# wesselb/stheno

Hardware: NVIDIA H100
Metric: log-marginal-likelihoods/sec (n=16384 fp64 EQ) (higher is better)
Workload: dtype f64

## Files before the change

stheno_b200/csrc/common.cuh:

```cuda
#pragma once
#include <cuda_runtime.h>
#include <stdint.h>

#include <atomic>
#include <mutex>

#include "../../include/gpk.h"

namespace gpk {

extern long long g_launch_count;

#define GPK_CHECK_LAUNCH()                                   \
  do {                                                       \
    cudaError_t e__ = cudaGetLastError();                    \
    if (e__ != cudaSuccess) return -1000 - (int)e__;         \
  } while (0)

#define GPK_COUNT_LAUNCH() (++::gpk::g_launch_count)

template <auto Kernel>
int opt_in_smem(int bytes) {
  static std::atomic<int> set[64];
  static std::mutex mu;
  int dev = 0;
  cudaError_t e = cudaGetDevice(&dev);
  if (e != cudaSuccess) return -1000 - (int)e;
  if (dev >= 64) return GPK_ERR_UNSUPPORTED;
  if (bytes <= set[dev].load(std::memory_order_acquire)) return 0;
  std::lock_guard<std::mutex> lock(mu);
  if (bytes <= set[dev].load(std::memory_order_relaxed)) return 0;
  e = cudaFuncSetAttribute(Kernel, cudaFuncAttributeMaxDynamicSharedMemorySize, bytes);
  if (e != cudaSuccess) return -1000 - (int)e;
  set[dev].store(bytes, std::memory_order_release);
  return 0;
}

__device__ __forceinline__ uint32_t smem_u32(const void* p) {
  return static_cast<uint32_t>(__cvta_generic_to_shared(p));
}

__device__ __forceinline__ void cp_async16(void* smem_dst, const void* gmem_src) {
  asm volatile("cp.async.cg.shared.global [%0], [%1], 16;\n" ::"r"(smem_u32(smem_dst)), "l"(gmem_src));
}
__device__ __forceinline__ void cp_async_commit() { asm volatile("cp.async.commit_group;\n" ::); }
template <int N>
__device__ __forceinline__ void cp_async_wait() {
  asm volatile("cp.async.wait_group %0;\n" ::"n"(N));
}

__device__ __forceinline__ void mbar_init(uint64_t* bar, uint32_t count) {
  asm volatile("mbarrier.init.shared::cta.b64 [%0], %1;\n" ::"r"(smem_u32(bar)), "r"(count));
}
__device__ __forceinline__ void fence_mbar_init() { asm volatile("fence.mbarrier_init.release.cluster;\n" ::); }
__device__ __forceinline__ void fence_proxy_async() { asm volatile("fence.proxy.async.shared::cta;\n" ::); }
__device__ __forceinline__ void mbar_arrive_expect_tx(uint64_t* bar, uint32_t bytes) {
  asm volatile("mbarrier.arrive.expect_tx.shared::cta.b64 _, [%0], %1;\n" ::"r"(smem_u32(bar)), "r"(bytes));
}
__device__ __forceinline__ void mbar_wait(uint64_t* bar, uint32_t phase) {
  asm volatile(
      "{\n"
      ".reg .pred P1;\n"
      "WAIT_LOOP:\n"
      "mbarrier.try_wait.parity.shared::cta.b64 P1, [%0], %1;\n"
      "@P1 bra WAIT_DONE;\n"
      "bra WAIT_LOOP;\n"
      "WAIT_DONE:\n"
      "}\n" ::"r"(smem_u32(bar)),
      "r"(phase)
      : "memory");
}
__device__ __forceinline__ void bulk_copy_g2s(void* smem_dst, const void* gmem_src, uint32_t bytes, uint64_t* bar) {
  asm volatile(
      "cp.async.bulk.shared::cluster.global.mbarrier::complete_tx::bytes [%0], [%1], %2, [%3];\n" ::"r"(
          smem_u32(smem_dst)),
      "l"(gmem_src), "r"(bytes), "r"(smem_u32(bar))
      : "memory");
}

__device__ __forceinline__ void dmma884(double& c0, double& c1, double a, double b) {
  asm("mma.sync.aligned.m8n8k4.row.col.f64.f64.f64.f64 {%0,%1}, {%2}, {%3}, {%0,%1};\n"
               : "+d"(c0), "+d"(c1)
               : "d"(a), "d"(b));
}

struct Emulation {
  int32_t slices = 0;
  void* scratch = nullptr;
  int64_t bytes = 0;
};
Emulation& emulation();

template <typename T>
__device__ __forceinline__ T warp_sum(T v) {
#pragma unroll
  for (int o = 16; o > 0; o >>= 1) v += __shfl_xor_sync(0xffffffffu, v, o);
  return v;
}

}
```

stheno_b200/csrc/gemm_oz.cu:

```cuda
#include <cuda.h>

#include "common.cuh"
#include "wgmma.cuh"

namespace gpk {
bool prof_enabled();
void prof_begin(cudaStream_t, double flops, int kind);
void prof_end(cudaStream_t);

namespace {

constexpr int OZ_BM = 128, OZ_BN = 64, OZ_BK = 64;
constexpr int OZ_HN = 32;
constexpr int OZ_THREADS = 384;

template <int S>
struct OzCfg {
  static constexpr bool PAD = S > 7;
  static constexpr int EXTRA = PAD ? 0 : S / 2;
  static constexpr int ACC = 16 * (S + EXTRA);
  static constexpr int RA = (192 - ACC) / 8 < S ? (192 - ACC) / 8 : S;
  static constexpr int A_SLICE = OZ_BM * OZ_BK;
  static constexpr int B_SLICE = OZ_HN * OZ_BK;
  static constexpr int A_BYTES = S * A_SLICE;
  static constexpr int Z_BYTES = PAD ? B_SLICE : 0;
  static constexpr int B_BYTES = S * B_SLICE;
  static constexpr int TX_BYTES = A_BYTES + B_BYTES;
  static constexpr int STAGE_BYTES = A_BYTES + Z_BYTES + B_BYTES;
  static constexpr int SMEM_MAX = 226 * 1024;
  static constexpr int STAGES = (SMEM_MAX - 1024) / STAGE_BYTES > 4 ? 4 : (SMEM_MAX - 1024) / STAGE_BYTES;
  static constexpr int SMEM_BYTES = STAGES * STAGE_BYTES + 1024;
  static_assert(STAGES >= 2, "ring");
};

struct OzParams {
  double alpha;
  double* C;
  const double* sc_a;
  const double* sc_b;
  int64_t ldc;
  int32_t a_row0, b_row0;
  int32_t KB, lower, tiles_m, tiles_n;
  int32_t total_tiles, tiles_per_cta, tri_rows;
  int32_t accumulate;
  int32_t band;
};

__device__ __forceinline__ void oz_mbar_wait(uint64_t* bar, uint32_t parity) {
  asm volatile(
      "{\n"
      ".reg .pred P1;\n"
      "OZW_LOOP:\n"
      "mbarrier.try_wait.parity.shared::cta.b64 P1, [%0], %1;\n"
      "@P1 bra OZW_DONE;\n"
      "bra OZW_LOOP;\n"
      "OZW_DONE:\n"
      "}\n" ::"r"(smem_u32(bar)),
      "r"(parity)
      : "memory");
}
__device__ __forceinline__ void oz_mbar_arrive(uint64_t* bar) {
  asm volatile("mbarrier.arrive.shared::cta.b64 _, [%0];\n" ::"r"(smem_u32(bar)) : "memory");
}
__device__ __forceinline__ void oz_tma_load_3d(void* dst, const CUtensorMap* map, int c0, int c1, int c2, uint64_t* bar) {
  asm volatile(
      "cp.async.bulk.tensor.3d.shared::cluster.global.mbarrier::complete_tx::bytes [%0], [%1, {%2, %3, %4}], [%5];\n" ::"r"(
          smem_u32(dst)),
      "l"(map), "r"(c0), "r"(c1), "r"(c2), "r"(smem_u32(bar))
      : "memory");
}
__device__ __forceinline__ double oz_i2d(uint32_t x) {
  return __hiloint2double(0x43300000, (int)(x ^ 0x80000000u)) - 4503601774854144.0;
}
template <int S, int SA, int N>
__device__ __forceinline__ void oz_wgmma(uint32_t* d, const uint32_t* a, uint32_t a_addr, uint32_t b_addr, uint32_t accumulate) {
  if constexpr (SA < OzCfg<S>::RA)
    wgmma_s8_ra<N>(d, a + 4 * SA, wgmma_desc<64>(b_addr), accumulate);
  else
    wgmma_s8<N>(d, wgmma_desc<64>(a_addr + SA * OzCfg<S>::A_SLICE), wgmma_desc<64>(b_addr), accumulate);
}
template <int S, int SA, int LO>
__device__ __forceinline__ void oz_mma_groups(uint32_t* acc, const uint32_t* a, uint32_t a_addr, uint32_t b_addr,
                                              uint32_t accumulate) {
  constexpr int W = S - LO < 2 ? S - LO : 2;
  oz_wgmma<S, SA, OZ_HN * W>(acc + 16 * LO, a, a_addr, b_addr + (LO - SA) * OzCfg<S>::B_SLICE, accumulate);
  if constexpr (LO + 2 < S) oz_mma_groups<S, SA, LO + 2>(acc, a, a_addr, b_addr, accumulate);
}
template <int S, int SA>
__device__ __forceinline__ void oz_mma_step(uint32_t* acc, const uint32_t* a, uint32_t a_addr, uint32_t b_addr,
                                            uint32_t accumulate) {
  using Cfg = OzCfg<S>;
  if constexpr (SA & 1) {
    if constexpr (Cfg::PAD)
      oz_wgmma<S, SA, 2 * OZ_HN>(acc + 16 * (SA - 1), a, a_addr, b_addr - Cfg::B_SLICE, 1u);
    else
      oz_wgmma<S, SA, OZ_HN>(acc + 16 * (S + SA / 2), a, a_addr, b_addr, accumulate);
  }
  constexpr int LO = (SA + 1) & ~1;
  if constexpr (LO < S) oz_mma_groups<S, SA, LO>(acc, a, a_addr, b_addr, SA == 0 ? accumulate : 1u);
  if constexpr (SA + 1 < S) oz_mma_step<S, SA + 1>(acc, a, a_addr, b_addr, accumulate);
}
__host__ __device__ __forceinline__ int oz_rows_before(const OzParams& p, int r) {
  if (!p.lower) return r * p.tiles_n;
  return r <= p.tri_rows ? r * (r + 1) : p.tri_rows * (p.tri_rows + 1) + (r - p.tri_rows) * p.tiles_n;
}
__host__ __device__ __forceinline__ void oz_tile(const OzParams& p, int t, int& tm, int& tn) {
  int r0 = 0;
  while (r0 + p.band < p.tiles_m && oz_rows_before(p, r0 + p.band) <= t) r0 += p.band;
  const int r1 = (r0 + p.band < p.tiles_m) ? r0 + p.band : p.tiles_m;
  int u = t - oz_rows_before(p, r0);
  const int nc0 = (p.lower && 2 * (r0 + 1) < p.tiles_n) ? 2 * (r0 + 1) : p.tiles_n;
  const int h = r1 - r0;
  if (u < nc0 * h) {
    tn = u / h;
    tm = r0 + (u - tn * h);
    return;
  }
  u -= nc0 * h;
  for (int c = nc0; c < p.tiles_n; ++c) {
    const int first = (c >> 1) > r0 ? (c >> 1) : r0;
    const int cnt = r1 - first;
    if (u < cnt) {
      tn = c;
      tm = first + u;
      return;
    }
    u -= cnt;
  }
  tm = r1 - 1;
  tn = p.tiles_n - 1;
}

template <int S>
__global__ void __launch_bounds__(OZ_THREADS, 1)
oz_gemm_kernel(const __grid_constant__ CUtensorMap mapA, const __grid_constant__ CUtensorMap mapB, const OzParams p) {
  using Cfg = OzCfg<S>;
  constexpr int STAGES = Cfg::STAGES;
  const int wg = threadIdx.x >> 7;
  const int t_begin = blockIdx.x * p.tiles_per_cta;
  const int t_end = min(t_begin + p.tiles_per_cta, p.total_tiles);

  extern __shared__ uint8_t oz_smem_raw[];
  uint8_t* smem = reinterpret_cast<uint8_t*>((reinterpret_cast<uintptr_t>(oz_smem_raw) + 1023) & ~uintptr_t(1023));
  __shared__ __align__(8) uint64_t full_bar[STAGES], empty_bar[STAGES];

  if (threadIdx.x == 0) {
    for (int s = 0; s < STAGES; ++s) {
      mbar_init(&full_bar[s], 1);
      mbar_init(&empty_bar[s], 256);
    }
    fence_mbar_init();
  }
  if constexpr (Cfg::PAD) {
    for (int i = threadIdx.x; i < STAGES * Cfg::Z_BYTES / 16; i += OZ_THREADS) {
      const int st = i / (Cfg::Z_BYTES / 16), j = i % (Cfg::Z_BYTES / 16);
      reinterpret_cast<uint4*>(smem + st * Cfg::STAGE_BYTES + Cfg::A_BYTES)[j] = make_uint4(0, 0, 0, 0);
    }
    asm volatile("fence.proxy.async.shared::cta;\n" ::: "memory");
  }
  __syncthreads();
  const int KB = p.KB;

  if (wg == 0) {
    asm volatile("setmaxnreg.dec.sync.aligned.u32 40;\n" ::);
    if (threadIdx.x == 0) {
      int g = 0;
      for (int t = t_begin; t < t_end; ++t) {
        int tm, tn;
        oz_tile(p, t, tm, tn);
        for (int h = 0; h < 2; ++h) {
          for (int kb = 0; kb < KB; ++kb, ++g) {
            const int s = g % STAGES, it = g / STAGES;
            if (it > 0) oz_mbar_wait(&empty_bar[s], (it - 1) & 1);
            uint8_t* st = smem + s * Cfg::STAGE_BYTES;
            mbar_arrive_expect_tx(&full_bar[s], Cfg::TX_BYTES);
            oz_tma_load_3d(st, &mapA, kb * OZ_BK, p.a_row0 + tm * OZ_BM, 0, &full_bar[s]);
            oz_tma_load_3d(st + Cfg::A_BYTES + Cfg::Z_BYTES, &mapB, kb * OZ_BK, p.b_row0 + tn * OZ_BN + h * OZ_HN, 0, &full_bar[s]);
          }
        }
      }
    }
    return;
  }
  asm volatile("setmaxnreg.inc.sync.aligned.u32 232;\n" ::);
  const int tid = threadIdx.x - 128 * wg, wrow = 64 * (wg - 1);
  const int r_lo = 16 * (tid >> 5) + ((tid & 31) >> 2), c_lo = 2 * (tid & 3);
  const double w_last = __hiloint2double((1023 - (12 + 7 * (S - 1))) << 20, 0);
  const int lane = tid & 31, a_row = wrow + 16 * (tid >> 5) + (lane & 7) + 8 * ((lane >> 3) & 1);
  const uint32_t a_off0 = a_row * OZ_BK + ((((lane >> 4) + 0) ^ ((lane >> 1) & 3)) << 4);
  const uint32_t a_off1 = a_row * OZ_BK + ((((lane >> 4) + 2) ^ ((lane >> 1) & 3)) << 4);
  uint32_t acc[Cfg::ACC];
  int g = 0;
  for (int t = t_begin; t < t_end; ++t) {
    int tm, tn;
    oz_tile(p, t, tm, tn);
    for (int h = 0; h < 2; ++h) {
      for (int kb = 0; kb < KB; ++kb, ++g) {
        const int s = g % STAGES, it = g / STAGES;
        oz_mbar_wait(&full_bar[s], it & 1);
        const uint32_t st = smem_u32(smem + s * Cfg::STAGE_BYTES), b0 = st + Cfg::A_BYTES + Cfg::Z_BYTES;
        uint32_t a[2][4 * Cfg::RA];
#pragma unroll
        for (int sl = 0; sl < Cfg::RA; ++sl) {
          ldmatrix_x4(a[0] + 4 * sl, st + sl * Cfg::A_SLICE + a_off0);
          ldmatrix_x4(a[1] + 4 * sl, st + sl * Cfg::A_SLICE + a_off1);
        }
        wgmma_fence();
#pragma unroll
        for (int ks = 0; ks < 2; ++ks)
          oz_mma_step<S, 0>(acc, a[ks], st + wrow * OZ_BK + ks * 32, b0 + ks * 32, (kb > 0 || ks > 0) ? 1u : 0u);
        wgmma_commit();
        wgmma_wait<0>();
        oz_mbar_arrive(&empty_bar[s]);
      }
      if constexpr (Cfg::EXTRA > 0) {
#pragma unroll
        for (int d = 1; d < S; d += 2)
#pragma unroll
          for (int i = 0; i < 16; ++i) acc[16 * d + i] += acc[16 * (S + d / 2) + i];
      }
      const int64_t row0 = (int64_t)tm * OZ_BM + wrow + r_lo;
      const int64_t col0 = (int64_t)tn * OZ_BN + h * OZ_HN + c_lo;
#pragma unroll
      for (int i = 0; i < 16; ++i) {
        const int64_t row = row0 + 8 * ((i >> 1) & 1), col = col0 + 8 * (i >> 2) + (i & 1);
        double v = oz_i2d(acc[i]);
#pragma unroll
        for (int d = 1; d < S; ++d) v = fma(v, 128.0, oz_i2d(acc[16 * d + i]));
        const double rs = p.alpha * w_last * __ldg(p.sc_a + row);
        const double out = v * (rs * __ldg(p.sc_b + col));
        double* c = p.C + row * p.ldc + col;
        if (p.accumulate)
          atomicAdd(c, out);
        else
          *c = out;
      }
    }
  }
}

template <int S>
__global__ void __launch_bounds__(256)
oz_slice_kernel(const double* __restrict__ P, int64_t ldp, int64_t rows, int32_t K, int8_t* __restrict__ planes,
                int64_t plane_stride, double* __restrict__ sc) {
  const int64_t row = (int64_t)blockIdx.x * 8 + (threadIdx.x >> 5);
  const int lane = threadIdx.x & 31;
  if (row >= rows) return;
  const double* src = P + row * ldp;
  double m = 0.0;
  for (int k = lane * 4; k < K; k += 128) {
    const double2 a = *reinterpret_cast<const double2*>(src + k), b = *reinterpret_cast<const double2*>(src + k + 2);
    m = fmax(fmax(fabs(a.x), fabs(a.y)), fmax(m, fmax(fabs(b.x), fabs(b.y))));
  }
#pragma unroll
  for (int o = 16; o > 0; o >>= 1) m = fmax(m, __shfl_xor_sync(0xffffffffu, m, o));
  int e = 0;
  if (m > 0.0 && m < 1e300) {
    e = ilogb(m) + 1;
    e = max(-1000, min(1000, e));
  }
  const double inv = __hiloint2double((1023 - e) << 20, 0);
  if (lane == 0) sc[row] = __hiloint2double((1023 + e) << 20, 0);
  int8_t* dst = planes + row * K;
  for (int k = lane * 4; k < K; k += 128) {
    const double2 a = *reinterpret_cast<const double2*>(src + k), b = *reinterpret_cast<const double2*>(src + k + 2);
    double r[4] = {a.x * inv, a.y * inv, b.x * inv, b.y * inv};
    double pw = 64.0, ipw = 1.0 / 64.0;
#pragma unroll
    for (int s = 0; s < S; ++s) {
      char4 q;
      double t;
      t = rint(r[0] * pw); r[0] = fma(-t, ipw, r[0]); q.x = (signed char)(int)t;
      t = rint(r[1] * pw); r[1] = fma(-t, ipw, r[1]); q.y = (signed char)(int)t;
      t = rint(r[2] * pw); r[2] = fma(-t, ipw, r[2]); q.z = (signed char)(int)t;
      t = rint(r[3] * pw); r[3] = fma(-t, ipw, r[3]); q.w = (signed char)(int)t;
      *reinterpret_cast<char4*>(dst + (int64_t)s * plane_stride + k) = q;
      pw *= 128.0;
      ipw *= 1.0 / 128.0;
    }
  }
}

typedef CUresult (*OzEncodeTiledFn)(CUtensorMap*, CUtensorMapDataType, cuuint32_t, void*, const cuuint64_t*,
                                    const cuuint64_t*, const cuuint32_t*, const cuuint32_t*, CUtensorMapInterleave,
                                    CUtensorMapSwizzle, CUtensorMapL2promotion, CUtensorMapFloatOOBfill);
OzEncodeTiledFn oz_encode_fn() {
  static OzEncodeTiledFn fn = [] {
    void* p = nullptr;
    cudaDriverEntryPointQueryResult q;
    if (cudaGetDriverEntryPoint("cuTensorMapEncodeTiled", &p, cudaEnableDefault, &q) != cudaSuccess)
      return (OzEncodeTiledFn) nullptr;
    return (OzEncodeTiledFn)p;
  }();
  return fn;
}

bool oz_make_map(CUtensorMap* m, const int8_t* planes, int64_t K, int64_t rows_cap, int64_t plane_stride, int S,
                 int box_rows) {
  OzEncodeTiledFn enc = oz_encode_fn();
  if (!enc) return false;
  cuuint64_t dims[3] = {(cuuint64_t)K, (cuuint64_t)rows_cap, (cuuint64_t)S};
  cuuint64_t strides[2] = {(cuuint64_t)K, (cuuint64_t)plane_stride};
  cuuint32_t box[3] = {(cuuint32_t)OZ_BK, (cuuint32_t)box_rows, (cuuint32_t)S};
  cuuint32_t es[3] = {1, 1, 1};
  return enc(m, CU_TENSOR_MAP_DATA_TYPE_UINT8, 3, const_cast<int8_t*>(planes), dims, strides, box, es,
             CU_TENSOR_MAP_INTERLEAVE_NONE, CU_TENSOR_MAP_SWIZZLE_64B, CU_TENSOR_MAP_L2_PROMOTION_L2_128B,
             CU_TENSOR_MAP_FLOAT_OOB_FILL_NONE) == CUDA_SUCCESS;
}

template <int S>
int oz_launch_slice(const double* P, int64_t ldp, int64_t rows, int64_t K, int8_t* planes, int64_t plane_stride, double* sc,
                    cudaStream_t stream) {
  if (rows == 0) return 0;
  oz_slice_kernel<S><<<(unsigned)((rows + 7) / 8), 256, 0, stream>>>(P, ldp, rows, (int32_t)K, planes, plane_stride, sc);
  GPK_COUNT_LAUNCH();
  cudaError_t e = cudaGetLastError();
  return e == cudaSuccess ? 0 : -1000 - (int)e;
}

__global__ void oz_scale_kernel(double* C, int64_t ldc, int64_t M, int64_t N, double beta) {
  const int64_t i = (int64_t)blockIdx.y, j = (int64_t)blockIdx.x * blockDim.x + threadIdx.x;
  if (i < M && j < N) C[i * ldc + j] *= beta;
}

template <int S>
int oz_launch_gemm(int64_t M, int64_t N, int64_t K, double alpha, const int8_t* planesA, int64_t capA, int64_t strideA,
                   const double* scA, int64_t rowA, const int8_t* planesB, int64_t capB, int64_t strideB,
                   const double* scB, int64_t rowB, double beta, double* C, int64_t ldc, int32_t lower,
                   cudaStream_t stream) {
  CUtensorMap mA, mB;
  if (!oz_make_map(&mA, planesA, K, capA, strideA, S, OZ_BM) || !oz_make_map(&mB, planesB, K, capB, strideB, S, OZ_HN))
    return GPK_ERR_UNSUPPORTED;
  if (const int rc = opt_in_smem<oz_gemm_kernel<S>>(OzCfg<S>::SMEM_BYTES)) return rc;
  if (beta != 0.0 && beta != 1.0) {
    if (M > 65535) return GPK_ERR_UNSUPPORTED;
    oz_scale_kernel<<<dim3((unsigned)((N + 255) / 256), (unsigned)M), 256, 0, stream>>>(C, ldc, M, N, beta);
    GPK_COUNT_LAUNCH();
  }
  const int32_t tiles_m = (int32_t)(M / OZ_BM), tiles_n = (int32_t)(N / OZ_BN);
  const int32_t tri_rows = lower ? (tiles_m < tiles_n / 2 ? tiles_m : tiles_n / 2) : 0;
  const int32_t total = lower ? tri_rows * (tri_rows + 1) + (tiles_m - tri_rows) * tiles_n : tiles_m * tiles_n;
  const int32_t tpc_cap = K > 512 ? 2 : 4;
  int32_t tpc = total / 264;
  tpc = tpc < 1 ? 1 : (tpc > tpc_cap ? tpc_cap : tpc);
  int32_t band = (int32_t)((12ll << 20) / (128ll * K * S));
  band = band < 1 ? 1 : (band > 16 ? 16 : band);
  OzParams p{alpha, C, scA + rowA, scB + rowB, ldc, (int32_t)rowA, (int32_t)rowB, (int32_t)(K / OZ_BK), lower,
             tiles_m, tiles_n, total, tpc, tri_rows, beta != 0.0 ? 1 : 0, band};
  if (prof_enabled()) prof_begin(stream, (double)total * 2.0 * OZ_BM * OZ_BN * (double)K, 1);
  oz_gemm_kernel<S><<<(unsigned)((total + tpc - 1) / tpc), OZ_THREADS, OzCfg<S>::SMEM_BYTES, stream>>>(mA, mB, p);
  if (prof_enabled()) prof_end(stream);
  GPK_COUNT_LAUNCH();
  cudaError_t e = cudaGetLastError();
  return e == cudaSuccess ? 0 : -1000 - (int)e;
}

}

int64_t oz_ws_bytes(int64_t rows, int64_t K, int32_t S) { return (int64_t)S * rows * K + rows * 8 + 256; }

static inline double* oz_scales(void* ws, int64_t rows, int64_t K, int32_t S) {
  const uintptr_t p = reinterpret_cast<uintptr_t>(ws) + (uintptr_t)((int64_t)S * rows * K);
  return reinterpret_cast<double*>((p + 255) & ~uintptr_t(255));
}

int oz_slice_panel(const double* P, int64_t ldp, int64_t rows, int64_t K, void* ws, int64_t cap_rows, int32_t S,
                   cudaStream_t stream) {
  if (K % 128 || K > 65536 || rows > cap_rows || ldp % 2 || reinterpret_cast<uintptr_t>(P) % 16) return GPK_ERR_ARG;
  int8_t* planes = static_cast<int8_t*>(ws);
  double* sc = oz_scales(ws, cap_rows, K, S);
  switch (S) {
    case 5: return oz_launch_slice<5>(P, ldp, rows, K, planes, cap_rows * K, sc, stream);
    case 6: return oz_launch_slice<6>(P, ldp, rows, K, planes, cap_rows * K, sc, stream);
    case 7: return oz_launch_slice<7>(P, ldp, rows, K, planes, cap_rows * K, sc, stream);
    case 8: return oz_launch_slice<8>(P, ldp, rows, K, planes, cap_rows * K, sc, stream);
  }
  return GPK_ERR_ARG;
}

int oz_gemm_sliced(int64_t M, int64_t N, int64_t K, double alpha, const void* wsA, int64_t capA, int64_t rowA,
                   const void* wsB, int64_t capB, int64_t rowB, double beta, double* C, int64_t ldc, int32_t lower,
                   int32_t S, cudaStream_t stream) {
  if (M % OZ_BM || N % OZ_BN || K % 128 || K > 65536 || ldc % 2 || reinterpret_cast<uintptr_t>(C) % 16) return GPK_ERR_ARG;
  if (M == 0 || N == 0) return 0;
  const int8_t* pa = static_cast<const int8_t*>(wsA);
  const int8_t* pb = static_cast<const int8_t*>(wsB);
  const double* sa = oz_scales(const_cast<void*>(wsA), capA, K, S);
  const double* sb = oz_scales(const_cast<void*>(wsB), capB, K, S);
#define OZ_CASE(SS)                                                                                                   \
  case SS:                                                                                                            \
    return oz_launch_gemm<SS>(M, N, K, alpha, pa, capA, capA * K, sa, rowA, pb, capB, capB * K, sb, rowB, beta, C, ldc, \
                              lower, stream);
  switch (S) {
    OZ_CASE(5)
    OZ_CASE(6)
    OZ_CASE(7)
    OZ_CASE(8)
  }
#undef OZ_CASE
  return GPK_ERR_ARG;
}

Emulation& emulation() {
  static thread_local Emulation em[64];
  int dev = 0;
  cudaGetDevice(&dev);
  return em[(dev < 0 || dev >= 64) ? 0 : dev];
}

static inline int64_t round_up_1k(int64_t x) { return (x + 1023) & ~int64_t(1023); }

int64_t oz_gemm_scratch_bytes(int64_t M, int64_t N, int64_t K, int32_t S) {
  return round_up_1k(oz_ws_bytes(M, K, S)) + oz_ws_bytes(N, K, S);
}

int gemm_nt_f64_emulated(int64_t M, int64_t N, int64_t K, double alpha, const double* A, int64_t lda, const double* B,
                         int64_t ldb, double beta, double* C, int64_t ldc, int32_t lower, cudaStream_t stream) {
  const Emulation& em = emulation();
  if (em.slices < 5 || em.slices > 8 || !em.scratch) return 0;
  if (M % OZ_BM || N % OZ_BN || K % 128 || lda % 2 || ldb % 2 || ldc % 2) return 0;
  if ((reinterpret_cast<uintptr_t>(A) | reinterpret_cast<uintptr_t>(B) | reinterpret_cast<uintptr_t>(C)) % 16) return 0;
  if (M < 256 || N < 256 || (double)M * (double)N * (double)K < 1.5e9) return 0;
  const bool same = (A == B && lda == ldb && M >= N);
  constexpr int64_t KC_MAX = 65536;
  const int64_t passes = (K + KC_MAX - 1) / KC_MAX;
  const int64_t kc = ((K / passes + 127) / 128) * 128;
  const int64_t off_b = same ? 0 : round_up_1k(oz_ws_bytes(M, kc, em.slices));
  if (em.bytes < off_b + oz_ws_bytes(same ? M : N, kc, em.slices)) return 0;
  int rc;
  void* wsa = em.scratch;
  void* wsb = static_cast<char*>(em.scratch) + off_b;
  for (int64_t k0 = 0; k0 < K; k0 += kc) {
    const int64_t kk = (K - k0 < kc) ? K - k0 : kc;
    if ((rc = oz_slice_panel(A + k0, lda, M, kk, wsa, M, em.slices, stream))) return rc;
    if (!same && (rc = oz_slice_panel(B + k0, ldb, N, kk, wsb, N, em.slices, stream))) return rc;
    if ((rc = oz_gemm_sliced(M, N, kk, alpha, wsa, M, 0, same ? wsa : wsb, same ? M : N, 0, k0 == 0 ? beta : 1.0, C, ldc, lower,
                             em.slices, stream)))
      return rc;
  }
  return 1;
}

}

extern "C" {

int gpk_set_f64_emulation(int32_t slices, void* scratch, int64_t scratch_bytes) {
  if (slices != 0 && (slices < 5 || slices > 8)) return GPK_ERR_ARG;
  if (slices != 0 && (!scratch || reinterpret_cast<uintptr_t>(scratch) % 1024 || scratch_bytes <= 0)) return GPK_ERR_ARG;
  gpk::Emulation& em = gpk::emulation();
  em.slices = slices;
  em.scratch = slices ? scratch : nullptr;
  em.bytes = slices ? scratch_bytes : 0;
  return 0;
}
int64_t gpk_f64_emulation_scratch_bytes(int64_t M, int64_t N, int64_t K, int32_t slices) {
  return gpk::oz_gemm_scratch_bytes(M, N, K, slices);
}

int64_t gpk_oz_ws_bytes(int64_t rows, int64_t K, int32_t slices) { return gpk::oz_ws_bytes(rows, K, slices); }

int32_t gpk_debug_oz_tile(int32_t lower, int32_t tiles_m, int32_t tiles_n, int32_t band, int32_t t, int32_t* tm, int32_t* tn) {
  gpk::OzParams p{};
  p.lower = lower;
  p.tiles_m = tiles_m;
  p.tiles_n = tiles_n;
  p.band = band;
  p.tri_rows = lower ? (tiles_m < tiles_n / 2 ? tiles_m : tiles_n / 2) : 0;
  p.total_tiles = lower ? p.tri_rows * (p.tri_rows + 1) + (tiles_m - p.tri_rows) * tiles_n : tiles_m * tiles_n;
  if (t >= 0 && t < p.total_tiles && tm && tn) {
    int a = 0, b = 0;
    gpk::oz_tile(p, t, a, b);
    *tm = a;
    *tn = b;
  }
  return p.total_tiles;
}

int gpk_gemm_nt_f64_oz(int64_t M, int64_t N, int64_t K, double alpha, const double* A, int64_t lda, const double* B,
                       int64_t ldb, double beta, double* C, int64_t ldc, int32_t lower, int32_t slices, void* ws,
                       int64_t ws_bytes, void* stream) {
  if (slices < 5 || slices > 8 || !ws) return GPK_ERR_ARG;
  const int64_t need_a = gpk::oz_ws_bytes(M, K, slices), need_b = gpk::oz_ws_bytes(N, K, slices);
  const bool same = (A == B && lda == ldb && M >= N);
  const int64_t off_b = same ? 0 : ((need_a + 1023) & ~int64_t(1023));
  if (ws_bytes < off_b + (same ? need_a : need_b) || reinterpret_cast<uintptr_t>(ws) % 1024) return GPK_ERR_ARG;
  cudaStream_t s = (cudaStream_t)stream;
  int rc;
  void* wsb = static_cast<char*>(ws) + off_b;
  if ((rc = gpk::oz_slice_panel(A, lda, M, K, ws, M, slices, s))) return rc;
  if (!same && (rc = gpk::oz_slice_panel(B, ldb, N, K, wsb, N, slices, s))) return rc;
  return gpk::oz_gemm_sliced(M, N, K, alpha, ws, M, 0, same ? ws : wsb, same ? M : N, 0, beta, C, ldc, lower, slices, s);
}

}
```

Before: 18.34.

## Split Ozaki GEMM tiles across 2-CTA clusters with multicast A loads

Launches the int8-sliced Ozaki GEMM as 2-CTA clusters. Each CTA computes one 32-column half of a 128x64 tile, and the A panel is loaded as two 64-row halves multicast to both CTAs. Consumers signal the empty barriers of both CTAs remotely, and the producer drains outstanding stages before exit. This replaces the old scheme where one CTA looped over both column halves and reloaded A for each. It is meant to halve A traffic per tile and double the number of CTAs working at once, at the cost of cross-CTA synchronisation and cluster scheduling constraints.

```diff
diff --git a/stheno_b200/csrc/common.cuh b/stheno_b200/csrc/common.cuh
--- a/stheno_b200/csrc/common.cuh
+++ b/stheno_b200/csrc/common.cuh
@@ -70,6 +70,32 @@
       "r"(phase)
       : "memory");
 }
+__device__ __forceinline__ uint32_t cluster_ctarank() {
+  uint32_t r;
+  asm volatile("mov.u32 %0, %%cluster_ctarank;\n" : "=r"(r));
+  return r;
+}
+__device__ __forceinline__ void cluster_sync() {
+  asm volatile("barrier.cluster.arrive.release;\nbarrier.cluster.wait.acquire;\n" ::: "memory");
+}
+__device__ __forceinline__ void mbar_arrive_cluster(uint64_t* bar, uint32_t rank) {
+  asm volatile(
+      "{\n"
+      ".reg .b32 remote;\n"
+      "mapa.shared::cluster.u32 remote, %0, %1;\n"
+      "mbarrier.arrive.shared::cluster.b64 _, [remote];\n"
+      "}\n" ::"r"(smem_u32(bar)),
+      "r"(rank)
+      : "memory");
+}
+__device__ __forceinline__ void tma_load_3d_multicast(void* dst, const void* map, int c0, int c1, int c2, uint64_t* bar,
+                                                      uint16_t cta_mask) {
+  asm volatile(
+      "cp.async.bulk.tensor.3d.shared::cluster.global.mbarrier::complete_tx::bytes.multicast::cluster [%0], [%1, {%2, %3, "
+      "%4}], [%5], %6;\n" ::"r"(smem_u32(dst)),
+      "l"(map), "r"(c0), "r"(c1), "r"(c2), "r"(smem_u32(bar)), "h"(cta_mask)
+      : "memory");
+}
 __device__ __forceinline__ void bulk_copy_g2s(void* smem_dst, const void* gmem_src, uint32_t bytes, uint64_t* bar) {
   asm volatile(
       "cp.async.bulk.shared::cluster.global.mbarrier::complete_tx::bytes [%0], [%1], %2, [%3];\n" ::"r"(
diff --git a/stheno_b200/csrc/gemm_oz.cu b/stheno_b200/csrc/gemm_oz.cu
--- a/stheno_b200/csrc/gemm_oz.cu
+++ b/stheno_b200/csrc/gemm_oz.cu
@@ -20,9 +20,10 @@
   static constexpr int EXTRA = PAD ? 0 : S / 2;
   static constexpr int ACC = 16 * (S + EXTRA);
   static constexpr int RA = (192 - ACC) / 8 < S ? (192 - ACC) / 8 : S;
-  static constexpr int A_SLICE = OZ_BM * OZ_BK;
+  static constexpr int A_SLICE = 64 * OZ_BK;
+  static constexpr int A_HALF = S * A_SLICE;
   static constexpr int B_SLICE = OZ_HN * OZ_BK;
-  static constexpr int A_BYTES = S * A_SLICE;
+  static constexpr int A_BYTES = 2 * A_HALF;
   static constexpr int Z_BYTES = PAD ? B_SLICE : 0;
   static constexpr int B_BYTES = S * B_SLICE;
   static constexpr int TX_BYTES = A_BYTES + B_BYTES;
@@ -59,8 +60,18 @@
       "r"(parity)
       : "memory");
 }
-__device__ __forceinline__ void oz_mbar_arrive(uint64_t* bar) {
-  asm volatile("mbarrier.arrive.shared::cta.b64 _, [%0];\n" ::"r"(smem_u32(bar)) : "memory");
+__device__ __forceinline__ void oz_mbar_wait_cluster(uint64_t* bar, uint32_t parity) {
+  asm volatile(
+      "{\n"
+      ".reg .pred P1;\n"
+      "OZC_LOOP:\n"
+      "mbarrier.try_wait.parity.acquire.cluster.shared::cta.b64 P1, [%0], %1;\n"
+      "@P1 bra OZC_DONE;\n"
+      "bra OZC_LOOP;\n"
+      "OZC_DONE:\n"
+      "}\n" ::"r"(smem_u32(bar)),
+      "r"(parity)
+      : "memory");
 }
 __device__ __forceinline__ void oz_tma_load_3d(void* dst, const CUtensorMap* map, int c0, int c1, int c2, uint64_t* bar) {
   asm volatile(
@@ -137,7 +148,8 @@
   using Cfg = OzCfg<S>;
   constexpr int STAGES = Cfg::STAGES;
   const int wg = threadIdx.x >> 7;
-  const int t_begin = blockIdx.x * p.tiles_per_cta;
+  const uint32_t rank = cluster_ctarank();
+  const int t_begin = (blockIdx.x >> 1) * p.tiles_per_cta;
   const int t_end = min(t_begin + p.tiles_per_cta, p.total_tiles);
 
   extern __shared__ uint8_t oz_smem_raw[];
@@ -147,7 +159,7 @@
   if (threadIdx.x == 0) {
     for (int s = 0; s < STAGES; ++s) {
       mbar_init(&full_bar[s], 1);
-      mbar_init(&empty_bar[s], 256);
+      mbar_init(&empty_bar[s], 2 * 8);
     }
     fence_mbar_init();
   }
@@ -158,7 +170,7 @@
     }
     asm volatile("fence.proxy.async.shared::cta;\n" ::: "memory");
   }
-  __syncthreads();
+  cluster_sync();
   const int KB = p.KB;
 
   if (wg == 0) {
@@ -168,33 +180,32 @@
       for (int t = t_begin; t < t_end; ++t) {
         int tm, tn;
         oz_tile(p, t, tm, tn);
-        for (int h = 0; h < 2; ++h) {
-          for (int kb = 0; kb < KB; ++kb, ++g) {
-            const int s = g % STAGES, it = g / STAGES;
-            if (it > 0) oz_mbar_wait(&empty_bar[s], (it - 1) & 1);
-            uint8_t* st = smem + s * Cfg::STAGE_BYTES;
-            mbar_arrive_expect_tx(&full_bar[s], Cfg::TX_BYTES);
-            oz_tma_load_3d(st, &mapA, kb * OZ_BK, p.a_row0 + tm * OZ_BM, 0, &full_bar[s]);
-            oz_tma_load_3d(st + Cfg::A_BYTES + Cfg::Z_BYTES, &mapB, kb * OZ_BK, p.b_row0 + tn * OZ_BN + h * OZ_HN, 0, &full_bar[s]);
-          }
+        for (int kb = 0; kb < KB; ++kb, ++g) {
+          const int s = g % STAGES, it = g / STAGES;
+          if (it > 0) oz_mbar_wait_cluster(&empty_bar[s], (it - 1) & 1);
+          uint8_t* st = smem + s * Cfg::STAGE_BYTES;
+          mbar_arrive_expect_tx(&full_bar[s], Cfg::TX_BYTES);
+          tma_load_3d_multicast(st + rank * Cfg::A_HALF, &mapA, kb * OZ_BK, p.a_row0 + tm * OZ_BM + 64 * rank, 0,
+                                &full_bar[s], 0x3);
+          oz_tma_load_3d(st + Cfg::A_BYTES + Cfg::Z_BYTES, &mapB, kb * OZ_BK, p.b_row0 + tn * OZ_BN + rank * OZ_HN, 0,
+                         &full_bar[s]);
         }
       }
+      for (int u = g > STAGES ? g - STAGES : 0; u < g; ++u) oz_mbar_wait_cluster(&empty_bar[u % STAGES], (u / STAGES) & 1);
     }
-    return;
-  }
-  asm volatile("setmaxnreg.inc.sync.aligned.u32 232;\n" ::);
-  const int tid = threadIdx.x - 128 * wg, wrow = 64 * (wg - 1);
-  const int r_lo = 16 * (tid >> 5) + ((tid & 31) >> 2), c_lo = 2 * (tid & 3);
-  const double w_last = __hiloint2double((1023 - (12 + 7 * (S - 1))) << 20, 0);
-  const int lane = tid & 31, a_row = wrow + 16 * (tid >> 5) + (lane & 7) + 8 * ((lane >> 3) & 1);
-  const uint32_t a_off0 = a_row * OZ_BK + ((((lane >> 4) + 0) ^ ((lane >> 1) & 3)) << 4);
-  const uint32_t a_off1 = a_row * OZ_BK + ((((lane >> 4) + 2) ^ ((lane >> 1) & 3)) << 4);
-  uint32_t acc[Cfg::ACC];
-  int g = 0;
-  for (int t = t_begin; t < t_end; ++t) {
-    int tm, tn;
-    oz_tile(p, t, tm, tn);
-    for (int h = 0; h < 2; ++h) {
+  } else {
+    asm volatile("setmaxnreg.inc.sync.aligned.u32 232;\n" ::);
+    const int tid = threadIdx.x - 128 * wg, half = wg - 1;
+    const int r_lo = 16 * (tid >> 5) + ((tid & 31) >> 2), c_lo = 2 * (tid & 3);
+    const double w_last = __hiloint2double((1023 - (12 + 7 * (S - 1))) << 20, 0);
+    const int lane = tid & 31, a_row = 16 * (tid >> 5) + (lane & 7) + 8 * ((lane >> 3) & 1);
+    const uint32_t a_off0 = half * Cfg::A_HALF + a_row * OZ_BK + ((((lane >> 4) + 0) ^ ((lane >> 1) & 3)) << 4);
+    const uint32_t a_off1 = half * Cfg::A_HALF + a_row * OZ_BK + ((((lane >> 4) + 2) ^ ((lane >> 1) & 3)) << 4);
+    uint32_t acc[Cfg::ACC];
+    int g = 0;
+    for (int t = t_begin; t < t_end; ++t) {
+      int tm, tn;
+      oz_tile(p, t, tm, tn);
       for (int kb = 0; kb < KB; ++kb, ++g) {
         const int s = g % STAGES, it = g / STAGES;
         oz_mbar_wait(&full_bar[s], it & 1);
@@ -208,10 +219,13 @@
         wgmma_fence();
 #pragma unroll
         for (int ks = 0; ks < 2; ++ks)
-          oz_mma_step<S, 0>(acc, a[ks], st + wrow * OZ_BK + ks * 32, b0 + ks * 32, (kb > 0 || ks > 0) ? 1u : 0u);
+          oz_mma_step<S, 0>(acc, a[ks], st + half * Cfg::A_HALF + ks * 32, b0 + ks * 32, (kb > 0 || ks > 0) ? 1u : 0u);
         wgmma_commit();
         wgmma_wait<0>();
-        oz_mbar_arrive(&empty_bar[s]);
+        if (lane == 0) {
+          mbar_arrive_cluster(&empty_bar[s], 0);
+          mbar_arrive_cluster(&empty_bar[s], 1);
+        }
       }
       if constexpr (Cfg::EXTRA > 0) {
 #pragma unroll
@@ -219,8 +233,8 @@
 #pragma unroll
           for (int i = 0; i < 16; ++i) acc[16 * d + i] += acc[16 * (S + d / 2) + i];
       }
-      const int64_t row0 = (int64_t)tm * OZ_BM + wrow + r_lo;
-      const int64_t col0 = (int64_t)tn * OZ_BN + h * OZ_HN + c_lo;
+      const int64_t row0 = (int64_t)tm * OZ_BM + 64 * half + r_lo;
+      const int64_t col0 = (int64_t)tn * OZ_BN + rank * OZ_HN + c_lo;
 #pragma unroll
       for (int i = 0; i < 16; ++i) {
         const int64_t row = row0 + 8 * ((i >> 1) & 1), col = col0 + 8 * (i >> 2) + (i & 1);
@@ -329,7 +343,7 @@
                    const double* scB, int64_t rowB, double beta, double* C, int64_t ldc, int32_t lower,
                    cudaStream_t stream) {
   CUtensorMap mA, mB;
-  if (!oz_make_map(&mA, planesA, K, capA, strideA, S, OZ_BM) || !oz_make_map(&mB, planesB, K, capB, strideB, S, OZ_HN))
+  if (!oz_make_map(&mA, planesA, K, capA, strideA, S, OZ_BM / 2) || !oz_make_map(&mB, planesB, K, capB, strideB, S, OZ_HN))
     return GPK_ERR_UNSUPPORTED;
   if (const int rc = opt_in_smem<oz_gemm_kernel<S>>(OzCfg<S>::SMEM_BYTES)) return rc;
   if (beta != 0.0 && beta != 1.0) {
@@ -341,15 +355,28 @@
   const int32_t tri_rows = lower ? (tiles_m < tiles_n / 2 ? tiles_m : tiles_n / 2) : 0;
   const int32_t total = lower ? tri_rows * (tri_rows + 1) + (tiles_m - tri_rows) * tiles_n : tiles_m * tiles_n;
   const int32_t tpc_cap = K > 512 ? 2 : 4;
-  int32_t tpc = total / 264;
+  int32_t tpc = total / 132;
   tpc = tpc < 1 ? 1 : (tpc > tpc_cap ? tpc_cap : tpc);
   int32_t band = (int32_t)((12ll << 20) / (128ll * K * S));
   band = band < 1 ? 1 : (band > 16 ? 16 : band);
   OzParams p{alpha, C, scA + rowA, scB + rowB, ldc, (int32_t)rowA, (int32_t)rowB, (int32_t)(K / OZ_BK), lower,
              tiles_m, tiles_n, total, tpc, tri_rows, beta != 0.0 ? 1 : 0, band};
   if (prof_enabled()) prof_begin(stream, (double)total * 2.0 * OZ_BM * OZ_BN * (double)K, 1);
-  oz_gemm_kernel<S><<<(unsigned)((total + tpc - 1) / tpc), OZ_THREADS, OzCfg<S>::SMEM_BYTES, stream>>>(mA, mB, p);
+  cudaLaunchAttribute cluster;
+  cluster.id = cudaLaunchAttributeClusterDimension;
+  cluster.val.clusterDim.x = 2;
+  cluster.val.clusterDim.y = 1;
+  cluster.val.clusterDim.z = 1;
+  cudaLaunchConfig_t cfg = {};
+  cfg.gridDim = dim3(2 * (unsigned)((total + tpc - 1) / tpc));
+  cfg.blockDim = dim3(OZ_THREADS);
+  cfg.dynamicSmemBytes = OzCfg<S>::SMEM_BYTES;
+  cfg.stream = stream;
+  cfg.attrs = &cluster;
+  cfg.numAttrs = 1;
+  const cudaError_t le = cudaLaunchKernelEx(&cfg, oz_gemm_kernel<S>, mA, mB, p);
   if (prof_enabled()) prof_end(stream);
+  if (le != cudaSuccess) return -1000 - (int)le;
   GPK_COUNT_LAUNCH();
   cudaError_t e = cudaGetLastError();
   return e == cudaSuccess ? 0 : -1000 - (int)e;
```

New measurement: 19.06, median of 6. 1.04x the previous value.
